# neuronest/custom-alphazero

Measured on AMD Instinct MI355X. Metric: self-play games/s (Connect-4 6x7, 100 sims/move), higher is better.
Workload: dtype fp32-accurate network (fp16 MFMA, two-term split operands, 3 products) / f64 PUCT

## Files before the change

custom-alphazero_amd/csrc/az_engine.hip:

```cpp
#include <math.h>
#include <string.h>

#include <stdio.h>
#include <stdlib.h>

#include <algorithm>
#include <map>
#include <string>
#include <vector>

#include "../../include/az.h"
#include "az_host.h"
#include "az_nn.h"
#include "az_tree.h"

namespace {

constexpr auto& fail = az::fail_abi;

int read_hw_queues() {
  const char* q = getenv("GPU_MAX_HW_QUEUES");
  const int v = q && *q ? atoi(q) : 0;
  return v > 0 ? v : 4;
}
// ... 79 lines not shown
  t.eval_count = base + 4 * K * p;
  t.miss_count = t.eval_count + K;
  t.nn_count = t.eval_count + 2 * K;
  t.next_counts = base + 4 * K * (p ^ 1);
}

void cells_from_board(const az::Board& b, int HW, int8_t* cells) {
  for (int c = 0; c < HW; ++c)
    cells[c] = az::bit(b.own, c) ? 1 : (az::bit(b.opp, c) ? -1 : 0);
}

int host_evaluate(az_engine* e, Lane& L, const az::Board* rows, const int32_t* n_rows) {
  hipStream_t s = L.stream;
  const int HW = L.g.HW, A = L.g.A;
  az::launch_encode(rows, n_rows, L.n, HW, L.x, s);
  AZ_HIP(hipGetLastError());
  AZ_HIP(hipMemcpyAsync(e->host_n, n_rows, sizeof(int32_t), hipMemcpyDeviceToHost, s));
  AZ_HIP(hipStreamSynchronize(s));
  const int n = *e->host_n;
  if (n <= 0) return 0;
  if (n > L.n) return fail(AZ_E_DEVICE, "host evaluator: leaf count past the lane's slots");
  AZ_HIP(hipMemcpyAsync(e->host_x, L.x, (size_t)n * HW * 4 * sizeof(float), hipMemcpyDeviceToHost, s));
  AZ_HIP(hipStreamSynchronize(s));
  if (e->host_fn(e->host_user, e->host_x, n, e->host_p, e->host_v) != 0)
    return fail(AZ_E_CALLBACK, "the host evaluator returned an error");
  AZ_HIP(hipMemcpyAsync(L.probs, e->host_p, (size_t)n * A * sizeof(float), hipMemcpyHostToDevice, s));
  AZ_HIP(hipMemcpyAsync(L.values, e->host_v, (size_t)n * sizeof(float), hipMemcpyHostToDevice, s));
  AZ_HIP(hipStreamSynchronize(s));
  return 0;
}

int sync_all(az_engine* e);

int simulate(az_engine* e, Lane& L) {
  hipStream_t s = L.stream;
  L.t.epoch += 1;
  if (++e->leaf_epoch == 0) {
    if (int rc = sync_all(e)) return rc;
    AZ_HIP(hipMemset(e->t.leaf_src, 0, (size_t)e->g.slots * sizeof(uint64_t)));
    e->leaf_epoch = 1;
  }
  L.t.leaf_epoch = e->leaf_epoch;
  set_counts(L.t, L.counts, L.t.epoch & 1);
  if (L.tree_timer.enabled) L.tree_timer.begin(s);
  az::launch_select(L.g, L.t, e->cache, s);
  if (L.tree_timer.enabled) L.tree_timer.end(s, 1);
  const az::Board* rows = L.t.eval_board;
  const int32_t* n_rows = L.t.eval_count;
  if (e->cache.enabled) {
    rows = L.t.nn_board;
    n_rows = L.t.nn_count;
  }
  if (e->cfg.evaluator == AZ_EVAL_NETWORK) {
    az::launch_forward(e->net, L.x, n_rows, L.n, L.g.H, L.g.W, L.g.A, L.act[0], L.act[1], L.act[2],
                       L.probs, L.values, s, L.timer.enabled ? &L.timer : nullptr, rows);
  } else if (e->cfg.evaluator == AZ_EVAL_HOST) {
    if (int rc = host_evaluate(e, L, rows, n_rows)) {
      e->broken = true;
      return rc;
    }
  } else {
    az::launch_synth_eval(L.g, rows, n_rows, L.probs, L.values, s);
  }
  if (L.tree_timer.enabled) L.tree_timer.begin(s);
  az::launch_expand(L.g, L.t, e->cache, L.probs, L.values, s);
  if (L.tree_timer.enabled) L.tree_timer.end(s, 1);
  AZ_HIP(hipGetLastError());
  return 0;
}

int sync_all(az_engine* e) {
  AZ_HIP(hipStreamSynchronize(e->stream));
  for (hipStream_t s : e->lane_streams) AZ_HIP(hipStreamSynchronize(s));
  if (e->own_pack_stream) AZ_HIP(hipStreamSynchronize(e->pack_stream));
  return 0;
}
// ... 1059 lines not shown
```

custom-alphazero_amd/csrc/az_tree.h:

```cpp
#pragma once
#include "az_device.h"

namespace az {

struct Edge {
  double W;
  double prior;
  int32_t N;
  int32_t child;
  int16_t child_n;
  int16_t action;
  float child_value;
};
static_assert(sizeof(Edge) == 32, "Edge must stay 32 bytes");

constexpr int kStatStride = 16;
enum : int {
  kStatExpansions = 0 * kStatStride,
  kStatTerminal = 1 * kStatStride,
  kStatGamesDone = 2 * kStatStride,
  kStatErrors = 3 * kStatStride,
  kStatSims = 4 * kStatStride,
  kStatPlies = 5 * kStatStride,
  kStatNextGame = 6 * kStatStride,
// ... 7 lines not shown
};
constexpr int kCountStride = 32;
constexpr int kCountWords = 2 * 4 * kCountStride;
enum : unsigned long long {
  kErrArena = 1, kErrPow = 2, kErrPath = 4, kErrIllegal = 8, kErrNoRoot = 16,
  kErrActRange = 32,
  kErrNoise = 64
};

constexpr int kPoolChunkA = 16;
struct TreeDev {
  Edge* edges;
  int32_t* arena_end;
  int32_t* slot_live;
  unsigned long long* pool_top;
  Edge* dst_edges;
  unsigned long long* dst_top;
  int32_t pool_cap;
  Board* root_board;
  int32_t* root_first;
  int32_t* root_n;
  float* root_value;
  int32_t* arena_top;
  int32_t* ply;
  int64_t* game_id;
  int32_t* path;
  int32_t* path_len;
  int32_t* slot_expansions;
  uint32_t* mt;
  int32_t mt_stride;
  uint64_t* leaf_src;
  Board* leaf_board;
  uint32_t leaf_epoch;
  Board* eval_board;
  int32_t* eval_count;
  int32_t* miss_count;
  Board* nn_board;
  int32_t* nn_count;
  int32_t* next_counts;
  uint32_t epoch;
  unsigned long long* stats;
  const double* powtab;
  int32_t* last_move;
  int32_t* last_status;
  double* last_policy;
  const double* noise_in;
  int32_t* noise_cur;
  int32_t noise_rows;
};

enum : uint32_t { kCacheEmpty = 0, kCacheClaimed = 1, kCacheReady = 2 };
constexpr uint32_t kCacheGenMask = 0x3fff;
constexpr uint32_t kCacheGenDiv = 16;
constexpr uint32_t kCacheEvictAge = 2;
AZ_HD uint32_t cache_fp(uint64_t h) { return (uint32_t)(h >> 48); }
AZ_HD uint32_t cache_age(uint32_t st, uint32_t gen) { return (gen - (st >> 2)) & kCacheGenMask; }
AZ_HD uint32_t cache_word(uint32_t fp, uint32_t gen, uint32_t status) {
  return (fp << 16) | ((gen & kCacheGenMask) << 2) | status;
}
struct CacheDev {
  Board* keys = nullptr;
  uint32_t* state = nullptr;
  float* pay = nullptr;
  uint32_t mask = 0;
  int enabled = 0;
  unsigned long long* ctl = nullptr;
// ... 46 lines not shown
```

custom-alphazero_amd/csrc/az_tree.hip:

```cpp
#include "az_random.h"
#include "az_tree.h"

namespace az {

constexpr int kGameBlock = 128;

__device__ __forceinline__ void stat_add(const TreeDev& t, int which, unsigned long long v) {
  atomicAdd(t.stats + which, v);
}

__device__ __forceinline__ int lane_id() { return (int)(threadIdx.x & 63); }
__device__ __forceinline__ int wave_claim(int32_t* counter) {
  const unsigned long long m = __ballot(1);
  const int leader = __ffsll((long long)m) - 1;
  const int rank = __popcll(m & ((1ull << lane_id()) - 1));
  int base = 0;
  if (lane_id() == leader) base = atomicAdd(counter, __popcll(m));
  return __shfl(base, leader) + rank;
}
__device__ __forceinline__ unsigned long long wave_claim64(unsigned long long* counter) {
  const unsigned long long m = __ballot(1);
  const int leader = __ffsll((long long)m) - 1;
  const int rank = __popcll(m & ((1ull << lane_id()) - 1));
  unsigned long long base = 0;
  if (lane_id() == leader) base = atomicAdd(counter, (unsigned long long)__popcll(m));
  return __shfl(base, leader) + (unsigned long long)rank;
}
__device__ __forceinline__ void wave_count(int32_t* counter) {
  const unsigned long long m = __ballot(1);
  if (lane_id() == __ffsll((long long)m) - 1) atomicAdd(counter, __popcll(m));
}
__device__ __forceinline__ void wave_stat(const TreeDev& t, int which, unsigned v = 1) {
  const unsigned long long m = __ballot(1);
  unsigned long long sum = 0;
#pragma unroll
  for (int bit = 0; bit < 8; ++bit) sum += (unsigned long long)__popcll(__ballot((v >> bit) & 1u)) << bit;
  if (lane_id() == __ffsll((long long)m) - 1 && sum) atomicAdd(t.stats + which, sum);
}
__device__ __forceinline__ void flag_error(const TreeDev& t, unsigned long long f) {
  atomicOr(t.stats + kStatErrors, f);
}

__device__ __forceinline__ void backup(Edge* E, const int32_t* __restrict__ path, int depth, double v) {
  constexpr int K = 8;
  for (int d1 = depth; d1 > 0; d1 -= K) {
    int id[K], n[K];
    double w[K];
#pragma unroll
    for (int k = 0; k < K; ++k)
      if (k < d1) id[k] = path[d1 - 1 - k];
#pragma unroll
    for (int k = 0; k < K; ++k)
      if (k < d1) {
        n[k] = E[id[k]].N;
        w[k] = E[id[k]].W;
      }
#pragma unroll
    for (int k = 0; k < K; ++k)
      if (k < d1) {
        E[id[k]].N = n[k] + 1;
        E[id[k]].W = w[k] + v;
        v = -v;
      }
  }
}

__device__ void mt_seed(const TreeDev& t, int slots, int g, uint32_t seed) {
  uint32_t prev = seed;
  t.mt[g] = seed;
  for (int i = 1; i < kMtN; ++i) {
    prev = 1812433253u * (prev ^ (prev >> 30)) + (uint32_t)i;
    t.mt[(size_t)i * slots + g] = prev;
  }
  t.mt[(size_t)kMtN * slots + g] = kMtN;
}

__device__ void mt_twist(uint32_t* m, size_t slots) {
  constexpr int kTwistB = 16;
  static_assert(kMtN % kTwistB == 0 && 227 >= kTwistB, "batches never read their own stores");
  uint32_t cur = m[0];
  for (int i0 = 0; i0 < kMtN; i0 += kTwistB) {
    uint32_t nx[kTwistB], far[kTwistB];
#pragma unroll
    for (int k = 0; k < kTwistB; ++k) {
      const int i = i0 + k;
      nx[k] = m[(size_t)(i + 1 < kMtN ? i + 1 : 0) * slots];
      far[k] = m[(size_t)(i + 397 < kMtN ? i + 397 : i - 227) * slots];
    }
#pragma unroll
    for (int k = 0; k < kTwistB; ++k) {
      const uint32_t y = (cur & 0x80000000u) | (nx[k] & 0x7fffffffu);
      m[(size_t)(i0 + k) * slots] = far[k] ^ (y >> 1) ^ ((y & 1u) ? 0x9908b0dfu : 0u);
      cur = nx[k];
    }
  }
}

// ... 39 lines not shown
    uint32_t* m = t.mt + s;
    const size_t slots = (size_t)t.mt_stride;
    uint32_t pos = kMtN;
    for (int n = g.rng_skip; n > 0;) {
      if (pos >= (uint32_t)kMtN) {
        mt_twist(m, slots);
        pos = 0;
      }
      const int k = min(n, kMtN - (int)pos);
      pos += (uint32_t)k;
      n -= k;
    }
    m[(size_t)kMtN * slots] = pos;
  }
}

#ifdef AZ_SEL_STAMPS
__device__ unsigned long long g_sel_stamps[16384][12];
#define AZ_SEL_ROW(s) ((((uintptr_t)(t.game_id + (s))) >> 3) & 16383)
#define AZ_SEL_STAMP(s, k) (g_sel_stamps[AZ_SEL_ROW(s)][k] = wall_clock64())
#define AZ_SEL_VALUE(s, k, v) (g_sel_stamps[AZ_SEL_ROW(s)][k] = (unsigned long long)(v))
extern "C" int az_diag_sel_stamps(unsigned long long* out, int n_slots) {
  return hipMemcpyFromSymbol(out, HIP_SYMBOL(g_sel_stamps), (size_t)std::min(n_slots, 16384) * 96) == hipSuccess ? 0 : -1;
}
#else
#define AZ_SEL_STAMP(s, k) ((void)0)
#define AZ_SEL_VALUE(s, k, v) ((void)0)
#endif
__device__ __forceinline__ bool same_board(const Board& a, const Board& b) {
  return a.own[0] == b.own[0] && a.own[1] == b.own[1] && a.opp[0] == b.opp[0] &&
         a.opp[1] == b.opp[1];
}

__device__ void leaf_tail(const GameCfg& g, const TreeDev& t, const CacheDev& c, int s, Edge* E,
                          const int32_t* path, int depth, int status, const Board& b) {
  wave_stat(t, kStatSims);
  wave_stat(t, kStatPathEdges, (unsigned)depth);
  AZ_SEL_STAMP(s, 3);
  if (depth > 0 && status != kOngoing) {
    backup(E, path, depth, status == kWin ? 1.0 : 0.0);
    wave_stat(t, kStatTerminal);
    return;
  }
  const uint64_t h = board_hash(b);
  uint32_t gen = 0, fp = 0, base = 0;
  uint32_t w[kCacheBucket];
  const uint64_t tag = (uint64_t)t.leaf_epoch << 32;
  t.leaf_board[s] = b;
  t.path_len[s] = depth;
  if (c.enabled) {
    gen = (uint32_t)__hip_atomic_load(c.ctl, __ATOMIC_RELAXED, __HIP_MEMORY_SCOPE_AGENT);
    fp = cache_fp(h);
    base = cache_bucket(c, h);
#pragma unroll
    for (int k = 0; k < kCacheBucket; ++k)
      w[k] = __hip_atomic_load(c.state + base + k, __ATOMIC_RELAXED, __HIP_MEMORY_SCOPE_AGENT);
  }
  AZ_SEL_STAMP(s, 4);
  if (!c.enabled) {
    const int q = wave_claim(t.eval_count);
    t.eval_board[q] = b;
    t.leaf_src[s] = tag | (uint32_t)(-(q + 1));
    wave_stat(t, kStatNNEvals);
    return;
  }
  {
    int hit = -1;
    uint32_t hst = 0;
    uint32_t cm = 0;
    bool stop = false;
#pragma unroll
    for (int k = 0; k < kCacheBucket; ++k) {
      const uint32_t st = w[k];
      if (stop) continue;
      if (st == kCacheEmpty) stop = true;
      else if ((st & 3u) == kCacheReady && (st >> 16) == fp) cm |= 1u << k;
    }
    if (cm) {
      __builtin_amdgcn_fence(__ATOMIC_ACQUIRE, "agent");
      for (; cm; cm &= cm - 1) {
        const int k = __builtin_ctz(cm);
        if (same_board(c.keys[base + k], b)) {
          hit = k;
#pragma unroll
          for (int kk = 0; kk < kCacheBucket; ++kk)
            if (kk == k) hst = w[kk];
          break;
        }
      }
    }
    bool use = hit >= 0;
    if (use && cache_age(hst, gen) != 0) {
      const uint32_t want = cache_word(fp, gen, kCacheReady);
      const uint32_t prev = atomicCAS(c.state + base + hit, hst, want);
      if (prev != hst) {
        __builtin_amdgcn_fence(__ATOMIC_ACQUIRE, "agent");
        use = prev == want && same_board(c.keys[base + hit], b);
      }
    }
    if (use) {
      const uint32_t idx = base + hit;
      t.leaf_src[s] = tag | idx;
      AZ_SEL_STAMP(s, 5);
      AZ_SEL_VALUE(s, 7, depth | (1 << 16) | ((uint64_t)s << 32));
      wave_stat(t, kStatCacheHits);
      return;
    }
  }
  AZ_SEL_STAMP(s, 5);
  AZ_SEL_VALUE(s, 7, depth | (2 << 16) | ((uint64_t)s << 32));
  wave_count(t.miss_count);
  const int row = wave_claim(t.nn_count);
  t.nn_board[row] = b;
  t.leaf_src[s] = tag | (uint32_t)(-(row + 1));
  wave_stat(t, kStatNNEvals);
}

struct SlotMt {
  const TreeDev* t;
  int s;
  __device__ uint32_t operator()() { return mt_next(*t, t->mt_stride, s); }
};
__device__ __forceinline__ double noisy_prior(const GameCfg& g, const Edge& e, double d) {
  const double kept = (e.action & kPrior64) ? (1.0 - g.noise_ratio) * e.prior
                                            : (double)((float)(1.0 - g.noise_ratio) * (float)e.prior);
  return kept + g.noise_ratio * d;
}
__device__ __forceinline__ bool argmax_before(double v, int i, double bv, int bi) {
  if (bv != bv) return v != v && i < bi;
  if (v != v) return true;
  return v > bv || (v == bv && i < bi);
}

template <bool NOISE>
__device__ __forceinline__ void select_body(const GameCfg& g, const TreeDev& t, const CacheDev& c) {
  if (blockIdx.x == 0 && threadIdx.x < 4) t.next_counts[threadIdx.x * kCountStride] = 0;
  const int s = blockIdx.x * blockDim.x + threadIdx.x;
  if (s >= g.slots || t.game_id[s] < 0) return;
  const BoardMasks mk = board_masks(g);
  Edge* E = slot_edges(g, t, s);
  int32_t* path = t.path + (size_t)s * g.max_depth;
  Board b = t.root_board[s];
  int first = t.root_first[s], cnt = t.root_n[s];
  int depth = 0, status = kOngoing;
  while (cnt > 0) {
    int sum = 0;
    for (int i = 0; i < cnt; ++i) sum += E[first + i].N;
// ... 28 lines not shown
        const double u = g.c_puct * noisy_prior(g, e, hn ? hn[i] : gam[i] * invacc) * sq / (double)(1 + e.N);
        const double ucb = q + u;
        if (i == 0 || argmax_before(ucb, i, best_v, best)) {
          best = i;
          best_v = ucb;
        }
      }
    } else {
      for (int i = 0; i < cnt; ++i) {
        const Edge e = E[first + i];
        const double q = e.N ? e.W / (double)e.N : 0.0;
        const double u = g.c_puct * e.prior * sq / (double)(1 + e.N);
        const double ucb = q + u;
        if (i == 0 || ucb > best_v) {
          best = i;
          best_v = ucb;
        }
      }
    }
    if (depth >= g.max_depth) {
      flag_error(t, kErrPath);
      return;
    }
    const Edge& e = E[first + best];
    path[depth++] = first + best;
    status = play_bb(g, mk, b, e.action & kActMask);
    if (status < 0) {
      flag_error(t, kErrIllegal);
      return;
    }
    first = e.child;
    cnt = e.child_n;
  }
  leaf_tail(g, t, c, s, E, path, depth, status, b);
}

template <int L, bool NOISE, int SHAPE>
__device__ __forceinline__ void select_group_body(const GameCfg& g, const TreeDev& t, const CacheDev& c) {
  if (blockIdx.x == 0 && threadIdx.x < 4) t.next_counts[threadIdx.x * kCountStride] = 0;
  const int gid = blockIdx.x * blockDim.x + threadIdx.x;
  const int s = gid / L, j = gid % L;
#ifdef AZ_SEL_STAMPS
  if (s < g.slots && j == 0) {
    AZ_SEL_STAMP(s, 0);
    for (int k = 1; k < 12; ++k) AZ_SEL_VALUE(s, k, 0);
  }
  unsigned long long ph_load = 0, ph_reduce = 0, ph_play = 0, ph_t = 0;
#define AZ_SEL_PHASE(acc)                   \
  do {                                      \
    __builtin_amdgcn_s_waitcnt(0);          \
    const unsigned long long now_ = wall_clock64(); \
    acc += now_ - ph_t;                     \
    ph_t = now_;                            \
  } while (0)
#else
#define AZ_SEL_PHASE(acc) ((void)0)
#endif
  if (s >= g.slots) return;
  const int64_t game = t.game_id[s];
  Board b = t.root_board[s];
  int first = t.root_first[s], cnt = t.root_n[s];
  if (game < 0) return;
  if (j == 0) AZ_SEL_STAMP(s, 1);
  const BoardMasks mk = board_masks(g);
  Edge* E = slot_edges(g, t, s);
  int32_t* path = t.path + (size_t)s * g.max_depth;
  int depth = 0, status = kOngoing;
  int sum_next = -1;
#ifdef AZ_SEL_STAMPS
  __builtin_amdgcn_s_waitcnt(0);
  if (j == 0) AZ_SEL_STAMP(s, 11);
#endif
  while (cnt > 0) {
#ifdef AZ_SEL_STAMPS
    ph_t = wall_clock64();
#endif
    const bool mine = j < cnt;
    double sq;
    int sum;
    if (sum_next >= 0) {
      sum = sum_next;
      if (sum >= g.pow_len) {
        if (j == 0) flag_error(t, kErrPow);
        return;
      }
      sq = t.powtab[sum];
    }
    Edge e;
    if (mine) e = E[first + j];
    if (sum_next < 0) {
      sum = mine ? e.N : 0;
#pragma unroll
      for (int off = L / 2; off > 0; off >>= 1) sum += __shfl_xor(sum, off, L);
      if (sum >= g.pow_len) {
        if (j == 0) flag_error(t, kErrPow);
        return;
      }
      sq = t.powtab[sum];
    }
    AZ_SEL_PHASE(ph_load);
// ... 37 lines not shown
        const int oj = __shfl_xor(best, off, L);
        if (argmax_before(ov, oj, best_v, best)) {
          best_v = ov;
          best = oj;
        }
      }
    } else {
      if (mine) {
        const double q = e.N ? e.W / (double)e.N : 0.0;
        const double u = g.c_puct * e.prior * sq / (double)(1 + e.N);
        best_v = q + u;
        best = j;
      }
#pragma unroll
      for (int off = L / 2; off > 0; off >>= 1) {
        const double ov = __shfl_xor(best_v, off, L);
        const int oj = __shfl_xor(best, off, L);
        if (ov > best_v || (ov == best_v && oj < best)) {
          best_v = ov;
          best = oj;
        }
      }
    }
    if (depth >= g.max_depth) {
      if (j == 0) flag_error(t, kErrPath);
      return;
    }
    const int action = __shfl(mine ? (int)(e.action & kActMask) : 0, best, L);
    const int child = __shfl(mine ? e.child : 0, best, L);
    const int child_n = __shfl(mine ? (int)e.child_n : 0, best, L);
    sum_next = __shfl(mine ? e.N : 0, best, L) - 1;
    AZ_SEL_PHASE(ph_reduce);
    if (j == 0) path[depth] = first + best;
    ++depth;
    if constexpr (SHAPE == 1) status = play_c64<6, 7, 4>(b, action);
    else status = play_bb(g, mk, b, action);
    AZ_SEL_PHASE(ph_play);
    if (status < 0) {
      if (j == 0) flag_error(t, kErrIllegal);
      return;
    }
    first = child;
    cnt = child_n;
  }
  if (j == 0) {
    AZ_SEL_STAMP(s, 2);
    AZ_SEL_VALUE(s, 8, ph_load);
    AZ_SEL_VALUE(s, 9, ph_reduce);
    AZ_SEL_VALUE(s, 10, ph_play);
    leaf_tail(g, t, c, s, E, path, depth, status, b);
    AZ_SEL_STAMP(s, 6);
  }
}

template <bool NOISE>
__global__ __launch_bounds__(kGameBlock) void select_kernel(GameCfg g, TreeDev t, CacheDev c) {
  select_body<NOISE>(g, t, c);
}
template <int L, bool NOISE, int SHAPE = 0>
__global__ __launch_bounds__(kGameBlock) void select_group_kernel(GameCfg g, TreeDev t, CacheDev c) {
  select_group_body<L, NOISE, SHAPE>(g, t, c);
}

__device__ void cache_insert_row(const GameCfg& g, const TreeDev& t, const CacheDev& c,
                                 const float* __restrict__ probs, const float* __restrict__ values, int u) {
  const int rows = *t.nn_count;
  if ((u - (int)threadIdx.x) >= rows) return;
  int idx = -1;
  uint32_t word = 0;
  bool was_empty = false;
  if (u < rows) {
    const Board b = t.nn_board[u];
    const uint64_t h = board_hash(b);
    const uint32_t gen = (uint32_t)__hip_atomic_load(c.ctl, __ATOMIC_RELAXED, __HIP_MEMORY_SCOPE_AGENT);
    const uint32_t fp = cache_fp(h);
    const uint32_t base = cache_bucket(c, h);
    uint32_t w[kCacheBucket];
#pragma unroll
    for (int k = 0; k < kCacheBucket; ++k)
      w[k] = __hip_atomic_load(c.state + base + k, __ATOMIC_RELAXED, __HIP_MEMORY_SCOPE_AGENT);
    uint32_t tried = 0;
    for (int attempt = 0; attempt < kCacheBucket && idx < 0; ++attempt) {
      int pick = -1;
// ... 33 lines not shown
    asm volatile("s_waitcnt vmcnt(0)" ::: "memory");
  }
  __syncthreads();
  if (idx < 0) return;
  atomicExch(c.state + idx, word);
  wave_stat(t, kStatCacheInserts);
  if (was_empty) wave_claim64(c.ctl + 2);
  const unsigned long long n = wave_claim64(c.ctl + 1) + 1;
  if (c.gen_size && n % c.gen_size == 0) atomicAdd(c.ctl, 1ull);
}

__global__ __launch_bounds__(256) void synth_eval_kernel(GameCfg g, const Board* __restrict__ boards,
                                                         const int32_t* __restrict__ count,
                                                         float* __restrict__ probs,
                                                         float* __restrict__ values) {
  const int i = blockIdx.x * blockDim.x + threadIdx.x;
  if (i >= *count) return;
  synth_eval(boards[i], g.A, probs + (size_t)i * g.A, values + i);
}

template <int MAXA, bool INSERT, int SHAPE = 0>
__global__ __launch_bounds__(kGameBlock) void expand_kernel(GameCfg g, TreeDev t, CacheDev c,
                                                     const float* __restrict__ probs,
                                                     const float* __restrict__ values, int exp_blocks) {
  if (INSERT && (int)blockIdx.x >= exp_blocks) {
    cache_insert_row(g, t, c, probs, values, ((int)blockIdx.x - exp_blocks) * blockDim.x + threadIdx.x);
    return;
  }
  const int s = blockIdx.x * blockDim.x + threadIdx.x;
  if (s >= g.slots) return;
  const uint64_t leaf = t.leaf_src[s];
  const Board b = t.leaf_board[s];
  Edge* E = slot_edges(g, t, s);
  const int top0 = t.arena_top[s];
  const int end0 = g.halves > 1 ? t.arena_end[s] : 0;
  const int live0 = g.halves > 1 ? t.slot_live[s] : 0;
  const int depth = t.path_len[s];
  const int exps = t.slot_expansions[s];
  const int32_t* path = t.path + (size_t)s * g.max_depth;
  constexpr int K = 8;
  int pv[K];
#pragma unroll
  for (int k = 0; k < K; ++k) pv[k] = k < g.max_depth ? path[k] : 0;
  if ((uint32_t)(leaf >> 32) != t.leaf_epoch) return;
  const int src = (int32_t)(uint32_t)leaf;
  const float* p;
  float v;
  if (src >= 0) {
    p = c.pay + (size_t)src * (g.A + 1);
    v = p[g.A];
  } else {
    const int row = -src - 1;
    p = probs + (size_t)row * g.A;
    v = values[row];
  }
  int pn[K];
  double pw[K];
#pragma unroll
  for (int k = 0; k < K; ++k)
    if (k < depth) {
      pn[k] = E[pv[k]].N;
      pw[k] = E[pv[k]].W;
    }
  float masked[MAXA];
  int moves[MAXA];
  int nl = 0, nm = 0;
  float sum = 0.0f;
  uint32_t legal = 0;
  if constexpr (SHAPE == 1) {
    static_assert(MAXA >= 7, "Connect-4 actions");
    legal = (uint32_t)(~(b.own[0] | b.opp[0])) & 0x7fu;
    float pa[7];
#pragma unroll
    for (int a = 0; a < 7; ++a) pa[a] = p[a];
#pragma unroll
    for (int a = 0; a < 7; ++a)
      if ((legal >> a) & 1u) sum += pa[a];
#pragma unroll
    for (int a = 0; a < 7; ++a) masked[a] = pa[a];
    nl = nm = __builtin_popcount(legal);
  } else {
    for (int a = 0; a < g.A; ++a)
      if (action_cell(g, b, a) >= 0) masked[nl++] = p[a];
    nm = moves_order(g, b, moves);
    sum = pairwise_sum_f32(masked, nl);
  }
  int first = top0;
  if (g.halves > 1) {
    int end = end0;
    if (first + nm > end) {
      const int ch = kPoolChunkA * g.A;
      const unsigned long long m = __ballot(1);
      const int leader = __ffsll((long long)m) - 1;
      const int rank = __popcll(m & ((1ull << lane_id()) - 1));
      unsigned long long base = 0;
      if (lane_id() == leader) base = atomicAdd(t.pool_top, (unsigned long long)__popcll(m) * ch);
      base = __shfl(base, leader) + (unsigned long long)rank * ch;
      if (base + ch > (unsigned long long)t.pool_cap) {
        flag_error(t, kErrArena);
        return;
      }
      first = (int)base;
      end = first + ch;
      t.arena_end[s] = end;
    }
    t.slot_live[s] = live0 + nm;
  } else if (first + nm > g.arena_cap) {
    flag_error(t, kErrArena);
    return;
  }
  if constexpr (SHAPE == 1) {
    int k = 0;
#pragma unroll
    for (int a = 0; a < 7; ++a)
      if ((legal >> a) & 1u) {
        Edge e;
        e.W = 0.0;
        e.prior = sum == 0.0f ? 1.0 / (double)nl : (double)(masked[a] / sum);
        e.N = 0;
        e.child = kNoChild;
        e.child_n = 0;
        e.action = (int16_t)(a | (sum == 0.0f ? kPrior64 : 0));
        e.child_value = 0.f;
        E[first + k] = e;
        ++k;
      }
  } else {
    for (int k = 0; k < nm; ++k) {
      Edge e;
      e.W = 0.0;
      e.prior = sum == 0.0f ? 1.0 / (double)nl : (double)(masked[k] / sum);
      e.N = 0;
      e.child = kNoChild;
      e.child_n = 0;
      e.action = (int16_t)(moves[k] | (sum == 0.0f ? kPrior64 : 0));
      e.child_value = 0.f;
      E[first + k] = e;
    }
  }
  t.arena_top[s] = first + nm;
  if (depth == 0) {
    t.root_first[s] = first;
    t.root_n[s] = nm;
    t.root_value[s] = v;
  } else {
    int pe_id = 0;
#pragma unroll
    for (int k = 0; k < K; ++k)
      if (k == depth - 1) pe_id = pv[k];
    if (depth > K) pe_id = path[depth - 1];
    Edge& pe = E[pe_id];
    pe.child = first;
    pe.child_n = (int16_t)nm;
    pe.child_value = v;
  }
  const double vb = -(double)v;
#pragma unroll
  for (int k = 0; k < K; ++k)
    if (k < depth) {
      E[pv[k]].N = pn[k] + 1;
      E[pv[k]].W = pw[k] + (((depth - 1 - k) & 1) ? -vb : vb);
    }
  if (depth > K) backup(E, path + K, depth - K, vb);
  t.slot_expansions[s] = exps + 1;
  wave_stat(t, kStatExpansions);
}

template <int MAXA>
__global__ __launch_bounds__(kGameBlock) void play_kernel(GameCfg g, TreeDev t, SampleDev smp,
                                                   const double* __restrict__ uniforms,
                                                   int greedy_mode, int deterministic, int refill) {
  const int s = blockIdx.x * blockDim.x + threadIdx.x;
  if (s >= g.slots || t.game_id[s] < 0) return;
  Edge* E = slot_edges(g, t, s);
  const int first = t.root_first[s], cnt = t.root_n[s];
  if (cnt <= 0) {
    flag_error(t, kErrNoRoot);
    return;
  }
  const int ply = t.ply[s];
  const bool greedy = greedy_mode < 0 ? ply >= g.greedy_ply : greedy_mode != 0;
  double pr[MAXA];
  if (greedy) {
    int best = 0;
    for (int i = 1; i < cnt; ++i)
      if (E[first + i].N > E[first + best].N) best = i;
    for (int i = 0; i < cnt; ++i) pr[i] = i == best ? 1.0 : 0.0;
  } else {
    double c[MAXA];
    for (int i = 0; i < cnt; ++i) c[i] = (double)E[first + i].N;
    const double sum = pairwise_sum_f64(c, cnt);
    for (int i = 0; i < cnt; ++i) pr[i] = sum == 0.0 ? 1.0 / (double)cnt : c[i] / sum;
  }
  int k;
  if (deterministic) {
    k = 0;
    for (int i = 1; i < cnt; ++i)
      if (pr[i] > pr[k]) k = i;
// ... 301 lines not shown
```

custom-alphazero_amd/custom_alphazero/engine.py:

```python
import ctypes
import os

import numpy as np

LIB_PATH = os.path.join(os.path.dirname(os.path.abspath(__file__)), "_lib", "libaz.so")

EVAL_NETWORK = 0
EVAL_SYNTHETIC = 1
EVAL_HOST = 2
CONV_F16X2 = 0
CONV_DIRECT = 1
CONV_F16X2_LAYERS = 2


class AzError(RuntimeError):
    pass


class Config(ctypes.Structure):
    _fields_ = [
        ("board_height", ctypes.c_int32), ("board_width", ctypes.c_int32),
        ("n", ctypes.c_int32), ("gravity", ctypes.c_int32),
        ("mcts_iterations", ctypes.c_int32), ("index_move_greedy", ctypes.c_int32),
        ("exploration_constant", ctypes.c_double), ("slots", ctypes.c_int32),
        ("evaluator", ctypes.c_int32), ("filters", ctypes.c_int32), ("depth", ctypes.c_int32),
        ("value_hidden", ctypes.c_int32), ("bn_epsilon", ctypes.c_double),
        ("arena_edges", ctypes.c_int64), ("max_tree_visits", ctypes.c_int64),
        ("cache_log2", ctypes.c_int32), ("conv_algo", ctypes.c_int32),
        ("lanes", ctypes.c_int32), ("compact", ctypes.c_int32),
        ("tower_natural_order", ctypes.c_int32), ("dirichlet_noise", ctypes.c_int32),
        ("dirichlet_alpha", ctypes.c_double), ("dirichlet_ratio", ctypes.c_double),
        ("rng_skip", ctypes.c_int32), ("reserved", ctypes.c_int32 * 1),
    ]


class ChessConfig(ctypes.Structure):
    _fields_ = [
        ("mcts_iterations", ctypes.c_int32), ("index_move_greedy", ctypes.c_int32),
        ("exploration_constant", ctypes.c_double), ("slots", ctypes.c_int32),
        ("evaluator", ctypes.c_int32), ("filters", ctypes.c_int32), ("depth", ctypes.c_int32),
        ("value_hidden", ctypes.c_int32), ("max_plies", ctypes.c_int32),
        ("bn_epsilon", ctypes.c_double), ("arena_edges", ctypes.c_int64),
        ("conv_algo", ctypes.c_int32), ("lanes", ctypes.c_int32), ("cache_log2", ctypes.c_int32),
        ("reserved", ctypes.c_int32 * 5),
    ]


class Tensor(ctypes.Structure):
    _fields_ = [("name", ctypes.c_char_p), ("data", ctypes.c_void_p), ("numel", ctypes.c_int64),
                ("on_device", ctypes.c_int32), ("reserved", ctypes.c_int32)]


class Stats(ctypes.Structure):
    _fields_ = [
        ("expansions", ctypes.c_int64), ("terminal_visits", ctypes.c_int64),
        ("games_done", ctypes.c_int64), ("simulations", ctypes.c_int64),
        ("plies", ctypes.c_int64), ("active_slots", ctypes.c_int64), ("errors", ctypes.c_int64),
        ("conv_launches", ctypes.c_int64), ("conv_ms", ctypes.c_double),
        ("cache_hits", ctypes.c_int64), ("evaluations", ctypes.c_int64),
        ("conv_busy_ms", ctypes.c_double), ("tree_launches", ctypes.c_int64), ("tree_ms", ctypes.c_double),
        ("path_edges", ctypes.c_int64), ("cache_inserts", ctypes.c_int64),
        ("cache_generation", ctypes.c_int64), ("cache_gen_size", ctypes.c_int64),
        ("cache_capacity", ctypes.c_int64), ("games_drained", ctypes.c_int64),
        ("max_retained", ctypes.c_int64), ("cache_entries", ctypes.c_int64),
        ("arena_edges", ctypes.c_int64), ("issued_flop_per_board", ctypes.c_double),
# ... 136 lines not shown
    return None if a is None else a.ctypes.data_as(ctypes.c_void_p)


def tensor_array(named):
    keep, items = [], []
    for name, t in named:
        on_dev = 0
        if hasattr(t, "is_cuda"):
            t = t.detach().float().contiguous()
            on_dev = int(t.is_cuda)
            if not on_dev:
                t = t.numpy()
        if on_dev:
            ptr, numel = t.data_ptr(), t.numel()
        else:
            t = np.ascontiguousarray(t, np.float32)
            ptr, numel = t.ctypes.data, t.size
        keep.append(t)
        items.append(Tensor(name.encode(), ptr, numel, on_dev, 0))
    arr = (Tensor * len(items))(*items)
    if any(i.on_device for i in items):
        import torch
        torch.cuda.synchronize()
    return arr, len(items), keep


class Engine:

    def __init__(self, height=6, width=7, n=4, gravity=True, mcts_iterations=100, slots=1,
                 evaluator=EVAL_NETWORK, index_move_greedy=8, exploration_constant=1.5,
                 filters=128, depth=4, value_hidden=256, bn_epsilon=1e-3, arena_edges=0,
                 max_tree_visits=0, device=0, cache_log2=0, conv_algo=CONV_F16X2,
                 lanes=0, compact=False, tower_natural_order=False, dirichlet_noise=False,
                 dirichlet_alpha=0.03, dirichlet_ratio=0.25, rng_skip=None):
        L = load_library()
        self.height, self.width, self.n, self.gravity = height, width, n, bool(gravity)
        self.action_space = width if gravity else width * height
        self.slots = slots
        self.mcts_iterations = mcts_iterations
        cfg = Config(board_height=height, board_width=width, n=n, gravity=int(bool(gravity)),
                     mcts_iterations=mcts_iterations, index_move_greedy=index_move_greedy,
                     exploration_constant=exploration_constant, slots=slots, evaluator=evaluator,
                     filters=filters, depth=depth, value_hidden=value_hidden,
                     bn_epsilon=bn_epsilon, arena_edges=arena_edges,
                     max_tree_visits=max_tree_visits, cache_log2=cache_log2, conv_algo=conv_algo,
                     lanes=lanes, compact=int(bool(compact)),
                     tower_natural_order=int(bool(tower_natural_order)),
                     dirichlet_noise=int(bool(dirichlet_noise)), dirichlet_alpha=float(dirichlet_alpha),
                     dirichlet_ratio=float(dirichlet_ratio),
                     rng_skip=2 * height * width * 4 if rng_skip is None else int(rng_skip))
        handle = ctypes.c_void_p()
        _check(L.az_engine_create(int(device), ctypes.byref(cfg), ctypes.byref(handle)))
        self._h = handle
        self._L = L
        self._n_games = 0
        self._host_fn = None
        self._host_error = None

    @property
    def lanes(self):
        return int(self._L.az_engine_lanes(self._h))

    def close(self):
        if getattr(self, "_h", None):
            self._L.az_engine_destroy(self._h)
            self._h = None

    def __del__(self):
        try:
            self.close()
        except Exception:
            pass

    def set_weights(self, named):
        arr, n, _keep = tensor_array(named)
        _check(self._L.az_engine_set_weights(self._h, arr, n))

    def set_host_evaluator(self, fn):
        H, W, A = self.height, self.width, self.action_space

        def cb(_user, xp, n, pp, vp):
            try:
                x = np.ctypeslib.as_array(xp, shape=(n, H, W, 4)).copy()
# ... 376 lines not shown
```

include/az.h:

```cpp
#ifndef AZ_H_
#define AZ_H_

#include <stdint.h>

#ifdef __cplusplus
extern "C" {
#endif

#define AZ_ABI_VERSION 10

#define AZ_OK 0
#define AZ_E_INVALID -1
#define AZ_E_HIP -2
#define AZ_E_STATE -3
#define AZ_E_DEVICE -4
#define AZ_E_CALLBACK -5

#define AZ_EVAL_NETWORK 0
#define AZ_EVAL_SYNTHETIC 1
#define AZ_EVAL_HOST 2

#define AZ_CONV_F16X2 0
#define AZ_CONV_DIRECT 1
#define AZ_CONV_F16X2_LAYERS 2

typedef struct az_engine az_engine;

typedef struct az_config {
    int32_t board_height;
    int32_t board_width;
    int32_t n;
    int32_t gravity;
    int32_t mcts_iterations;
    int32_t index_move_greedy;
    double exploration_constant;
    int32_t slots;
    int32_t evaluator;
    int32_t filters;
    int32_t depth;
    int32_t value_hidden;
    double bn_epsilon;
    int64_t arena_edges;
    int64_t max_tree_visits;
    int32_t cache_log2;
    int32_t conv_algo;
    int32_t lanes;
    int32_t compact;
    int32_t tower_natural_order;
    int32_t dirichlet_noise;
    double dirichlet_alpha;
    double dirichlet_ratio;
    int32_t rng_skip;
    int32_t reserved[1];
} az_config;

typedef struct az_tensor {
    const char* name;
    const float* data;
    int64_t numel;
    int32_t on_device;
    int32_t reserved;
} az_tensor;

typedef struct az_stats {
    int64_t expansions;
    int64_t terminal_visits;
    int64_t games_done;
    int64_t simulations;
    int64_t plies;
    int64_t active_slots;
    int64_t errors;
    int64_t conv_launches;
    double conv_ms;
    int64_t cache_hits;
    int64_t evaluations;
    double conv_busy_ms;
    int64_t tree_launches;
    double tree_ms;
    int64_t path_edges;
    int64_t cache_inserts;
    int64_t cache_generation;
    int64_t cache_gen_size;
    int64_t cache_capacity;
    int64_t games_drained;
    int64_t max_retained;
    int64_t cache_entries;
// ... 70 lines not shown
```

Baseline: 10990.

## Expand cache-hit leaves directly inside the select kernel

When the evaluation cache is on and the action count is small, select now loads the cached policy/value payload during the bucket probe. On a hit it performs the expansion and backup in place, instead of recording the leaf for a later expand kernel. The shared expansion logic moves into a header so select and expand can both use it. The aim is to avoid a round-trip through global memory and the per-leaf work in a separate launch for cache hits. The cost is more registers and payload loads in the select kernel, including speculative loads on every probed key, which may lower occupancy.

Result: no change. 10970 (-0.2%).

```diff
diff --git a/custom-alphazero_amd/csrc/az_engine.hip b/custom-alphazero_amd/csrc/az_engine.hip
--- a/custom-alphazero_amd/csrc/az_engine.hip
+++ b/custom-alphazero_amd/csrc/az_engine.hip
@@ -135,6 +135,8 @@
 
 int sync_all(az_engine* e);
 
+bool expand_hits_in_select(int expand_launch, int A) { return expand_launch == 0 && A >= 1 && A <= 16; }
+
 int simulate(az_engine* e, Lane& L) {
   hipStream_t s = L.stream;
   L.t.epoch += 1;
@@ -145,6 +147,7 @@
   }
   L.t.leaf_epoch = e->leaf_epoch;
   set_counts(L.t, L.counts, L.t.epoch & 1);
+  L.t.fuse_hits = expand_hits_in_select(e->cfg.expand_launch, L.g.A);
   if (L.tree_timer.enabled) L.tree_timer.begin(s);
   az::launch_select(L.g, L.t, e->cache, s);
   if (L.tree_timer.enabled) L.tree_timer.end(s, 1);
diff --git a/custom-alphazero_amd/csrc/az_expand.h b/custom-alphazero_amd/csrc/az_expand.h
--- /dev/null
+++ b/custom-alphazero_amd/csrc/az_expand.h
@@ -0,0 +1,186 @@
+#pragma once
+#include "az_tree.h"
+
+namespace az {
+
+__device__ __forceinline__ int lane_id() { return (int)(threadIdx.x & 63); }
+__device__ __forceinline__ void wave_stat(const TreeDev& t, int which, unsigned v = 1) {
+  const unsigned long long m = __ballot(1);
+  unsigned long long sum = 0;
+#pragma unroll
+  for (int bit = 0; bit < 8; ++bit) sum += (unsigned long long)__popcll(__ballot((v >> bit) & 1u)) << bit;
+  if (lane_id() == __ffsll((long long)m) - 1 && sum) atomicAdd(t.stats + which, sum);
+}
+__device__ __forceinline__ void flag_error(const TreeDev& t, unsigned long long f) {
+  atomicOr(t.stats + kStatErrors, f);
+}
+
+__device__ __forceinline__ void backup(Edge* E, const int32_t* __restrict__ path, int depth, double v) {
+#pragma clang fp contract(off)
+  constexpr int K = 8;
+  for (int d1 = depth; d1 > 0; d1 -= K) {
+    int id[K], n[K];
+    double w[K];
+#pragma unroll
+    for (int k = 0; k < K; ++k)
+      if (k < d1) id[k] = path[d1 - 1 - k];
+#pragma unroll
+    for (int k = 0; k < K; ++k)
+      if (k < d1) {
+        n[k] = E[id[k]].N;
+        w[k] = E[id[k]].W;
+      }
+#pragma unroll
+    for (int k = 0; k < K; ++k)
+      if (k < d1) {
+        E[id[k]].N = n[k] + 1;
+        E[id[k]].W = w[k] + v;
+        v = -v;
+      }
+  }
+}
+
+constexpr int kExpandAhead = 8;
+struct ExpandSlot {
+  int top0, end0, live0, exps;
+  int pv[kExpandAhead];
+  int pn[kExpandAhead];
+  double pw[kExpandAhead];
+};
+__device__ __forceinline__ void expand_load_slot(const GameCfg& g, const TreeDev& t, int s, ExpandSlot& x) {
+  x.top0 = t.arena_top[s];
+  x.end0 = g.halves > 1 ? t.arena_end[s] : 0;
+  x.live0 = g.halves > 1 ? t.slot_live[s] : 0;
+  x.exps = t.slot_expansions[s];
+}
+__device__ __forceinline__ void expand_load_path(const GameCfg& g, const int32_t* path, ExpandSlot& x) {
+#pragma unroll
+  for (int k = 0; k < kExpandAhead; ++k) x.pv[k] = k < g.max_depth ? path[k] : 0;
+}
+__device__ __forceinline__ void expand_load_edges(const Edge* E, int depth, ExpandSlot& x) {
+#pragma unroll
+  for (int k = 0; k < kExpandAhead; ++k)
+    if (k < depth) {
+      x.pn[k] = E[x.pv[k]].N;
+      x.pw[k] = E[x.pv[k]].W;
+    }
+}
+
+template <int MAXA, int SHAPE>
+__device__ __forceinline__ bool expand_apply(const GameCfg& g, const TreeDev& t, int s, Edge* E,
+                                             const int32_t* path, int depth, const Board& b,
+                                             const ExpandSlot& x, const float* p, float v, float* masked,
+                                             int* moves) {
+#pragma clang fp contract(off)
+  constexpr int K = kExpandAhead;
+  int nl = 0, nm = 0;
+  float sum = 0.0f;
+  uint32_t legal = 0;
+  float pa[7];
+  if constexpr (SHAPE == 1) {
+    static_assert(MAXA >= 7, "Connect-4 actions");
+    legal = (uint32_t)(~(b.own[0] | b.opp[0])) & 0x7fu;
+#pragma unroll
+    for (int a = 0; a < 7; ++a) pa[a] = p[a];
+#pragma unroll
+    for (int a = 0; a < 7; ++a)
+      if ((legal >> a) & 1u) sum += pa[a];
+    nl = nm = __builtin_popcount(legal);
+  } else {
+    if constexpr (MAXA <= 16) {
+      float pl[MAXA];
+#pragma unroll
+      for (int a = 0; a < MAXA; ++a) pl[a] = a < g.A ? p[a] : 0.f;
+#pragma unroll
+      for (int a = 0; a < MAXA; ++a)
+        if (a < g.A && action_cell(g, b, a) >= 0) masked[nl++] = pl[a];
+    } else {
+      for (int a = 0; a < g.A; ++a)
+        if (action_cell(g, b, a) >= 0) masked[nl++] = p[a];
+    }
+    nm = moves_order(g, b, moves);
+    sum = pairwise_sum_f32(masked, nl);
+  }
+  int first = x.top0;
+  if (g.halves > 1) {
+    int end = x.end0;
+    if (first + nm > end) {
+      const int ch = kPoolChunkA * g.A;
+      const unsigned long long m = __ballot(1);
+      const int leader = __ffsll((long long)m) - 1;
+      const int rank = __popcll(m & ((1ull << lane_id()) - 1));
+      unsigned long long base = 0;
+      if (lane_id() == leader) base = atomicAdd(t.pool_top, (unsigned long long)__popcll(m) * ch);
+      base = __shfl(base, leader) + (unsigned long long)rank * ch;
+      if (base + ch > (unsigned long long)t.pool_cap) {
+        flag_error(t, kErrArena);
+        return false;
+      }
+      first = (int)base;
+      end = first + ch;
+      t.arena_end[s] = end;
+    }
+    t.slot_live[s] = x.live0 + nm;
+  } else if (first + nm > g.arena_cap) {
+    flag_error(t, kErrArena);
+    return false;
+  }
+  if constexpr (SHAPE == 1) {
+    int k = 0;
+#pragma unroll
+    for (int a = 0; a < 7; ++a)
+      if ((legal >> a) & 1u) {
+        Edge e;
+        e.W = 0.0;
+        e.prior = sum == 0.0f ? 1.0 / (double)nl : (double)(pa[a] / sum);
+        e.N = 0;
+        e.child = kNoChild;
+        e.child_n = 0;
+        e.action = (int16_t)(a | (sum == 0.0f ? kPrior64 : 0));
+        e.child_value = 0.f;
+        E[first + k] = e;
+        ++k;
+      }
+  } else {
+    for (int k = 0; k < nm; ++k) {
+      Edge e;
+      e.W = 0.0;
+      e.prior = sum == 0.0f ? 1.0 / (double)nl : (double)(masked[k] / sum);
+      e.N = 0;
+      e.child = kNoChild;
+      e.child_n = 0;
+      e.action = (int16_t)(moves[k] | (sum == 0.0f ? kPrior64 : 0));
+      e.child_value = 0.f;
+      E[first + k] = e;
+    }
+  }
+  t.arena_top[s] = first + nm;
+  if (depth == 0) {
+    t.root_first[s] = first;
+    t.root_n[s] = nm;
+    t.root_value[s] = v;
+  } else {
+    int pe_id = 0;
+#pragma unroll
+    for (int k = 0; k < K; ++k)
+      if (k == depth - 1) pe_id = x.pv[k];
+    if (depth > K) pe_id = path[depth - 1];
+    Edge& pe = E[pe_id];
+    pe.child = first;
+    pe.child_n = (int16_t)nm;
+    pe.child_value = v;
+  }
+  const double vb = -(double)v;
+#pragma unroll
+  for (int k = 0; k < K; ++k)
+    if (k < depth) {
+      E[x.pv[k]].N = x.pn[k] + 1;
+      E[x.pv[k]].W = x.pw[k] + (((depth - 1 - k) & 1) ? -vb : vb);
+    }
+  if (depth > K) backup(E, path + K, depth - K, vb);
+  t.slot_expansions[s] = x.exps + 1;
+  wave_stat(t, kStatExpansions);
+  return true;
+}
+
+}
diff --git a/custom-alphazero_amd/csrc/az_tree.h b/custom-alphazero_amd/csrc/az_tree.h
--- a/custom-alphazero_amd/csrc/az_tree.h
+++ b/custom-alphazero_amd/csrc/az_tree.h
@@ -63,6 +63,7 @@
   uint64_t* leaf_src;
   Board* leaf_board;
   uint32_t leaf_epoch;
+  int32_t fuse_hits;
   Board* eval_board;
   int32_t* eval_count;
   int32_t* miss_count;
diff --git a/custom-alphazero_amd/csrc/az_tree.hip b/custom-alphazero_amd/csrc/az_tree.hip
--- a/custom-alphazero_amd/csrc/az_tree.hip
+++ b/custom-alphazero_amd/csrc/az_tree.hip
@@ -1,4 +1,5 @@
 #include "az_random.h"
+#include "az_expand.h"
 #include "az_tree.h"
 
 namespace az {
@@ -9,7 +10,6 @@
   atomicAdd(t.stats + which, v);
 }
 
-__device__ __forceinline__ int lane_id() { return (int)(threadIdx.x & 63); }
 __device__ __forceinline__ int wave_claim(int32_t* counter) {
   const unsigned long long m = __ballot(1);
   const int leader = __ffsll((long long)m) - 1;
@@ -29,40 +29,6 @@
 __device__ __forceinline__ void wave_count(int32_t* counter) {
   const unsigned long long m = __ballot(1);
   if (lane_id() == __ffsll((long long)m) - 1) atomicAdd(counter, __popcll(m));
-}
-__device__ __forceinline__ void wave_stat(const TreeDev& t, int which, unsigned v = 1) {
-  const unsigned long long m = __ballot(1);
-  unsigned long long sum = 0;
-#pragma unroll
-  for (int bit = 0; bit < 8; ++bit) sum += (unsigned long long)__popcll(__ballot((v >> bit) & 1u)) << bit;
-  if (lane_id() == __ffsll((long long)m) - 1 && sum) atomicAdd(t.stats + which, sum);
-}
-__device__ __forceinline__ void flag_error(const TreeDev& t, unsigned long long f) {
-  atomicOr(t.stats + kStatErrors, f);
-}
-
-__device__ __forceinline__ void backup(Edge* E, const int32_t* __restrict__ path, int depth, double v) {
-  constexpr int K = 8;
-  for (int d1 = depth; d1 > 0; d1 -= K) {
-    int id[K], n[K];
-    double w[K];
-#pragma unroll
-    for (int k = 0; k < K; ++k)
-      if (k < d1) id[k] = path[d1 - 1 - k];
-#pragma unroll
-    for (int k = 0; k < K; ++k)
-      if (k < d1) {
-        n[k] = E[id[k]].N;
-        w[k] = E[id[k]].W;
-      }
-#pragma unroll
-    for (int k = 0; k < K; ++k)
-      if (k < d1) {
-        E[id[k]].N = n[k] + 1;
-        E[id[k]].W = w[k] + v;
-        v = -v;
-      }
-  }
 }
 
 __device__ void mt_seed(const TreeDev& t, int slots, int g, uint32_t seed) {
@@ -168,8 +134,10 @@
          a.opp[1] == b.opp[1];
 }
 
+template <int MAXA, int SHAPE>
 __device__ void leaf_tail(const GameCfg& g, const TreeDev& t, const CacheDev& c, int s, Edge* E,
-                          const int32_t* path, int depth, int status, const Board& b) {
+                          const int32_t* path, int depth, int status, const Board& b,
+                          const int (&pv)[kExpandAhead]) {
   wave_stat(t, kStatSims);
   wave_stat(t, kStatPathEdges, (unsigned)depth);
   AZ_SEL_STAMP(s, 3);
@@ -182,8 +150,21 @@
   uint32_t gen = 0, fp = 0, base = 0;
   uint32_t w[kCacheBucket];
   const uint64_t tag = (uint64_t)t.leaf_epoch << 32;
-  t.leaf_board[s] = b;
-  t.path_len[s] = depth;
+  auto leaf_record = [&](uint32_t src) {
+    t.leaf_board[s] = b;
+    t.path_len[s] = depth;
+    t.leaf_src[s] = tag | src;
+  };
+  const bool fuse = MAXA > 0 && t.fuse_hits && c.enabled;
+  ExpandSlot xs;
+  if constexpr (MAXA > 0) {
+    if (fuse) {
+      expand_load_slot(g, t, s, xs);
+#pragma unroll
+      for (int k = 0; k < kExpandAhead; ++k) xs.pv[k] = pv[k];
+      expand_load_edges(E, depth, xs);
+    }
+  }
   if (c.enabled) {
     gen = (uint32_t)__hip_atomic_load(c.ctl, __ATOMIC_RELAXED, __HIP_MEMORY_SCOPE_AGENT);
     fp = cache_fp(h);
@@ -196,13 +177,20 @@
   if (!c.enabled) {
     const int q = wave_claim(t.eval_count);
     t.eval_board[q] = b;
-    t.leaf_src[s] = tag | (uint32_t)(-(q + 1));
+    leaf_record((uint32_t)(-(q + 1)));
     wave_stat(t, kStatNNEvals);
     return;
   }
   {
     int hit = -1;
     uint32_t hst = 0;
+    constexpr int kPay = MAXA == 0 ? 1 : SHAPE == 1 ? 8 : MAXA + 1;
+    float pay[kPay];
+    auto load_payload = [&](uint32_t idx) {
+      const float* pp = c.pay + (size_t)idx * (SHAPE == 1 ? 8 : g.A + 1);
+#pragma unroll
+      for (int a = 0; a < kPay; ++a) pay[a] = SHAPE == 1 || a <= g.A ? pp[a] : 0.f;
+    };
     uint32_t cm = 0;
     bool stop = false;
 #pragma unroll
@@ -216,7 +204,11 @@
       __builtin_amdgcn_fence(__ATOMIC_ACQUIRE, "agent");
       for (; cm; cm &= cm - 1) {
         const int k = __builtin_ctz(cm);
-        if (same_board(c.keys[base + k], b)) {
+        const Board kb = c.keys[base + k];
+        if constexpr (kPay > 1) {
+          if (fuse) load_payload(base + k);
+        }
+        if (same_board(kb, b)) {
           hit = k;
 #pragma unroll
           for (int kk = 0; kk < kCacheBucket; ++kk)
@@ -232,14 +224,33 @@
       if (prev != hst) {
         __builtin_amdgcn_fence(__ATOMIC_ACQUIRE, "agent");
         use = prev == want && same_board(c.keys[base + hit], b);
+        if constexpr (kPay > 1) {
+          if (use && fuse) load_payload(base + hit);
+        }
       }
     }
     if (use) {
       const uint32_t idx = base + hit;
-      t.leaf_src[s] = tag | idx;
       AZ_SEL_STAMP(s, 5);
       AZ_SEL_VALUE(s, 7, depth | (1 << 16) | ((uint64_t)s << 32));
       wave_stat(t, kStatCacheHits);
+      if constexpr (MAXA > 0) {
+        if (fuse) {
+          if constexpr (SHAPE == 1) {
+            expand_apply<MAXA, 1>(g, t, s, E, path, depth, b, xs, pay, pay[7], nullptr, nullptr);
+          } else {
+            float v = 0.f;
+#pragma unroll
+            for (int a = 1; a < kPay; ++a)
+              if (a == g.A) v = pay[a];
+            float masked[MAXA];
+            int moves[MAXA];
+            expand_apply<MAXA, 0>(g, t, s, E, path, depth, b, xs, pay, v, masked, moves);
+          }
+          return;
+        }
+      }
+      leaf_record(idx);
       return;
     }
   }
@@ -248,7 +259,7 @@
   wave_count(t.miss_count);
   const int row = wave_claim(t.nn_count);
   t.nn_board[row] = b;
-  t.leaf_src[s] = tag | (uint32_t)(-(row + 1));
+  leaf_record((uint32_t)(-(row + 1)));
   wave_stat(t, kStatNNEvals);
 }
 
@@ -343,7 +354,8 @@
     first = e.child;
     cnt = e.child_n;
   }
-  leaf_tail(g, t, c, s, E, path, depth, status, b);
+  const int no_pv[kExpandAhead] = {};
+  leaf_tail<0, 0>(g, t, c, s, E, path, depth, status, b, no_pv);
 }
 
 template <int L, bool NOISE, int SHAPE>
@@ -377,6 +389,7 @@
   Edge* E = slot_edges(g, t, s);
   int32_t* path = t.path + (size_t)s * g.max_depth;
   int depth = 0, status = kOngoing;
+  int pv[kExpandAhead] = {};
   int sum_next = -1;
 #ifdef AZ_SEL_STAMPS
   __builtin_amdgcn_s_waitcnt(0);
@@ -480,6 +493,9 @@
     sum_next = __shfl(mine ? e.N : 0, best, L) - 1;
     AZ_SEL_PHASE(ph_reduce);
     if (j == 0) path[depth] = first + best;
+#pragma unroll
+    for (int k = 0; k < kExpandAhead; ++k)
+      if (k == depth) pv[k] = first + best;
     ++depth;
     if constexpr (SHAPE == 1) status = play_c64<6, 7, 4>(b, action);
     else status = play_bb(g, mk, b, action);
@@ -496,7 +512,7 @@
     AZ_SEL_VALUE(s, 8, ph_load);
     AZ_SEL_VALUE(s, 9, ph_reduce);
     AZ_SEL_VALUE(s, 10, ph_play);
-    leaf_tail(g, t, c, s, E, path, depth, status, b);
+    leaf_tail<(L <= 16 ? 16 : 0), SHAPE>(g, t, c, s, E, path, depth, status, b, pv);
     AZ_SEL_STAMP(s, 6);
   }
 }
@@ -596,16 +612,11 @@
   const uint64_t leaf = t.leaf_src[s];
   const Board b = t.leaf_board[s];
   Edge* E = slot_edges(g, t, s);
-  const int top0 = t.arena_top[s];
-  const int end0 = g.halves > 1 ? t.arena_end[s] : 0;
-  const int live0 = g.halves > 1 ? t.slot_live[s] : 0;
+  ExpandSlot x;
+  expand_load_slot(g, t, s, x);
   const int depth = t.path_len[s];
-  const int exps = t.slot_expansions[s];
   const int32_t* path = t.path + (size_t)s * g.max_depth;
-  constexpr int K = 8;
-  int pv[K];
-#pragma unroll
-  for (int k = 0; k < K; ++k) pv[k] = k < g.max_depth ? path[k] : 0;
+  expand_load_path(g, path, x);
   if ((uint32_t)(leaf >> 32) != t.leaf_epoch) return;
   const int src = (int32_t)(uint32_t)leaf;
   const float* p;
@@ -618,116 +629,10 @@
     p = probs + (size_t)row * g.A;
     v = values[row];
   }
-  int pn[K];
-  double pw[K];
-#pragma unroll
-  for (int k = 0; k < K; ++k)
-    if (k < depth) {
-      pn[k] = E[pv[k]].N;
-      pw[k] = E[pv[k]].W;
-    }
-  float masked[MAXA];
-  int moves[MAXA];
-  int nl = 0, nm = 0;
-  float sum = 0.0f;
-  uint32_t legal = 0;
-  if constexpr (SHAPE == 1) {
-    static_assert(MAXA >= 7, "Connect-4 actions");
-    legal = (uint32_t)(~(b.own[0] | b.opp[0])) & 0x7fu;
-    float pa[7];
-#pragma unroll
-    for (int a = 0; a < 7; ++a) pa[a] = p[a];
-#pragma unroll
-    for (int a = 0; a < 7; ++a)
-      if ((legal >> a) & 1u) sum += pa[a];
-#pragma unroll
-    for (int a = 0; a < 7; ++a) masked[a] = pa[a];
-    nl = nm = __builtin_popcount(legal);
-  } else {
-    for (int a = 0; a < g.A; ++a)
-      if (action_cell(g, b, a) >= 0) masked[nl++] = p[a];
-    nm = moves_order(g, b, moves);
-    sum = pairwise_sum_f32(masked, nl);
-  }
-  int first = top0;
-  if (g.halves > 1) {
-    int end = end0;
-    if (first + nm > end) {
-      const int ch = kPoolChunkA * g.A;
-      const unsigned long long m = __ballot(1);
-      const int leader = __ffsll((long long)m) - 1;
-      const int rank = __popcll(m & ((1ull << lane_id()) - 1));
-      unsigned long long base = 0;
-      if (lane_id() == leader) base = atomicAdd(t.pool_top, (unsigned long long)__popcll(m) * ch);
-      base = __shfl(base, leader) + (unsigned long long)rank * ch;
-      if (base + ch > (unsigned long long)t.pool_cap) {
-        flag_error(t, kErrArena);
-        return;
-      }
-      first = (int)base;
-      end = first + ch;
-      t.arena_end[s] = end;
-    }
-    t.slot_live[s] = live0 + nm;
-  } else if (first + nm > g.arena_cap) {
-    flag_error(t, kErrArena);
-    return;
-  }
-  if constexpr (SHAPE == 1) {
-    int k = 0;
-#pragma unroll
-    for (int a = 0; a < 7; ++a)
-      if ((legal >> a) & 1u) {
-        Edge e;
-        e.W = 0.0;
-        e.prior = sum == 0.0f ? 1.0 / (double)nl : (double)(masked[a] / sum);
-        e.N = 0;
-        e.child = kNoChild;
-        e.child_n = 0;
-        e.action = (int16_t)(a | (sum == 0.0f ? kPrior64 : 0));
-        e.child_value = 0.f;
-        E[first + k] = e;
-        ++k;
-      }
-  } else {
-    for (int k = 0; k < nm; ++k) {
-      Edge e;
-      e.W = 0.0;
-      e.prior = sum == 0.0f ? 1.0 / (double)nl : (double)(masked[k] / sum);
-      e.N = 0;
-      e.child = kNoChild;
-      e.child_n = 0;
-      e.action = (int16_t)(moves[k] | (sum == 0.0f ? kPrior64 : 0));
-      e.child_value = 0.f;
-      E[first + k] = e;
-    }
-  }
-  t.arena_top[s] = first + nm;
-  if (depth == 0) {
-    t.root_first[s] = first;
-    t.root_n[s] = nm;
-    t.root_value[s] = v;
-  } else {
-    int pe_id = 0;
-#pragma unroll
-    for (int k = 0; k < K; ++k)
-      if (k == depth - 1) pe_id = pv[k];
-    if (depth > K) pe_id = path[depth - 1];
-    Edge& pe = E[pe_id];
-    pe.child = first;
-    pe.child_n = (int16_t)nm;
-    pe.child_value = v;
-  }
-  const double vb = -(double)v;
-#pragma unroll
-  for (int k = 0; k < K; ++k)
-    if (k < depth) {
-      E[pv[k]].N = pn[k] + 1;
-      E[pv[k]].W = pw[k] + (((depth - 1 - k) & 1) ? -vb : vb);
-    }
-  if (depth > K) backup(E, path + K, depth - K, vb);
-  t.slot_expansions[s] = exps + 1;
-  wave_stat(t, kStatExpansions);
+  expand_load_edges(E, depth, x);
+  float masked[SHAPE == 1 ? 1 : MAXA];
+  int moves[SHAPE == 1 ? 1 : MAXA];
+  expand_apply<MAXA, SHAPE>(g, t, s, E, path, depth, b, x, p, v, masked, moves);
 }
 
 template <int MAXA>
diff --git a/custom-alphazero_amd/custom_alphazero/engine.py b/custom-alphazero_amd/custom_alphazero/engine.py
--- a/custom-alphazero_amd/custom_alphazero/engine.py
+++ b/custom-alphazero_amd/custom_alphazero/engine.py
@@ -30,7 +30,7 @@
         ("lanes", ctypes.c_int32), ("compact", ctypes.c_int32),
         ("tower_natural_order", ctypes.c_int32), ("dirichlet_noise", ctypes.c_int32),
         ("dirichlet_alpha", ctypes.c_double), ("dirichlet_ratio", ctypes.c_double),
-        ("rng_skip", ctypes.c_int32), ("reserved", ctypes.c_int32 * 1),
+        ("rng_skip", ctypes.c_int32), ("expand_launch", ctypes.c_int32),
     ]
 
 
@@ -233,7 +233,7 @@
                  filters=128, depth=4, value_hidden=256, bn_epsilon=1e-3, arena_edges=0,
                  max_tree_visits=0, device=0, cache_log2=0, conv_algo=CONV_F16X2,
                  lanes=0, compact=False, tower_natural_order=False, dirichlet_noise=False,
-                 dirichlet_alpha=0.03, dirichlet_ratio=0.25, rng_skip=None):
+                 dirichlet_alpha=0.03, dirichlet_ratio=0.25, rng_skip=None, expand_launch=False):
         L = load_library()
         self.height, self.width, self.n, self.gravity = height, width, n, bool(gravity)
         self.action_space = width if gravity else width * height
@@ -249,7 +249,8 @@
                      tower_natural_order=int(bool(tower_natural_order)),
                      dirichlet_noise=int(bool(dirichlet_noise)), dirichlet_alpha=float(dirichlet_alpha),
                      dirichlet_ratio=float(dirichlet_ratio),
-                     rng_skip=2 * height * width * 4 if rng_skip is None else int(rng_skip))
+                     rng_skip=2 * height * width * 4 if rng_skip is None else int(rng_skip),
+                     expand_launch=int(bool(expand_launch)))
         handle = ctypes.c_void_p()
         _check(L.az_engine_create(int(device), ctypes.byref(cfg), ctypes.byref(handle)))
         self._h = handle
diff --git a/include/az.h b/include/az.h
--- a/include/az.h
+++ b/include/az.h
@@ -51,7 +51,7 @@
     double dirichlet_alpha;
     double dirichlet_ratio;
     int32_t rng_skip;
-    int32_t reserved[1];
+    int32_t expand_launch;
 } az_config;
 
 typedef struct az_tensor {
```
